# guangkun0818/speech2text

Measured on AMD Instinct MI355X. Metric: audio-seconds/sec (train step, zipformer pruned-RNN-T), higher is better.
Workload: dtype f32; 1 GPU; C3 zipformer pruned-RNN-T train step: chunk_size -1, 500 BPE, prune_range 5 (fbank+fwd+bwd+allreduce+ScaledAdam); accumulate_grad_batches=1, gemm_arith=bf16x2/3, per_gpu_batch=64, global_batch=64, labels_per_utt=50, parallelism=dp1

## Files before the change

include/s2t_mi355.h:

```cpp
#ifndef S2T_MI355_H_
#define S2T_MI355_H_

#ifdef __cplusplus
extern "C" {
#endif

int s2t_fbank_f32(const float* pcm, long pcm_stride, const long* num_samples, int batch,
                  const float* window400, const float* twiddle512, const int* mel_off,
                  const int* mel_k0, const float* mel_w, int nnz, int num_mel, float eps,
                  float scale_in, const float* cmvn_mean, const float* cmvn_istd, float* out,
                  int max_frames, long* out_frames, void* stream);

#define S2T_FBANK_CARRY_MAX 559
#define S2T_FBANK_STATE_LONGS 4
int s2t_fbank_chunk_max_frames(long chunk_samples);
int s2t_fbank_chunk_f32(const float* pcm, long pcm_stride, const long* chunk_samples, const int* flush,
                        int batch, float* carry, long* counts, const float* window400,
                        const float* twiddle512, const int* mel_off, const int* mel_k0,
                        const float* mel_w, int nnz, int num_mel, float eps, float scale_in,
                        const float* cmvn_mean, const float* cmvn_istd, float* out, int max_new_frames,
                        long* new_frames, void* stream);

#define S2T_CTC_MAX_LABELS 1023
long s2t_ctc_workspace_floats(int B, int T, int Umax);
// ... 698 lines not shown
int s2t_gemm_x3p_bal(const float* A, long lda, const unsigned short* Bp, int N, int K, float* C, long ldc,
                     int M, const float* resid, long ldr, const float* act_src, long ld_act, int act_kind,
                     int tile, float* bal_stats, float min_mean, float max_mean, float min_rms,
                     float max_rms, float grad_scale, void* stream);

typedef struct S2tRowMap {
  int hw, w;
  long sb, sh, sw, base;
} S2tRowMap;
int s2t_gemm_x3p_map(const float* A, const S2tRowMap* amap, int seg, int nseg, const long* segoff,
                     const unsigned short* Bp, int N, float* C, long ldc, const S2tRowMap* cmap,
                     long c_elems, int M, const float* bias, int tile, void* stream);

void* s2t_side_stream(void);
int s2t_stream_order(void* from, void* to);

int s2t_x3p_sample_begin(int every);
int s2t_x3p_sample_end(long* launches, double* total_ms, double* bytes, double* flops);
int s2t_x3p_sample_min_bytes(double* bytes_min);
long s2t_gemm_x3p_calls(void);
long s2t_linear_lt_calls(void);
int s2t_prof_pair_create(void** start, void** stop);
int s2t_prof_pair_arm(void* start, void* stop);
int s2t_prof_pair_consumed(void);
int s2t_prof_pair_ms(void* start, void* stop, float* ms);
int s2t_prof_pair_destroy(void* start, void* stop);


int s2t_add_f32(const float* a, const float* b, float* out, long n, void* stream);
int s2t_balancer_next_parity(void);

int s2t_bmm_lt(int mode, const float* A, const float* B, float* C, int batch, int M, int N, int K,
               void* workspace, long ws_bytes, void* stream);

#define S2T_ZL_NDEC 32
#define S2T_ZL_NWHITEN 11
typedef struct S2tZlLin {
  const float* w;
  const float* b;
  float* gw;
  float* gb;
  const unsigned short* pf;
  const unsigned short* pb;
  int N, K;
} S2tZlLin;
typedef struct S2tZlBal {
  float min_mean, max_mean, min_rms, max_rms, grad_scale;
} S2tZlBal;
typedef struct S2tZlWh {
  int groups;
  float limit, grad_scale;
} S2tZlWh;
typedef struct S2tZlFf {
  S2tZlLin in, out;
  S2tZlBal hidden;
  S2tZlWh out_wh;
  S2tZlBal post;
} S2tZlFf;
typedef struct S2tZlSa {
  S2tZlLin in, out;
  S2tZlWh wh;
} S2tZlSa;
typedef struct S2tZlConv {
  S2tZlLin in, out;
  S2tZlBal bal1, bal2;
  S2tZlWh wh;
// ... 86 lines not shown
```

speech2text_amd/csrc/gemm.hip:

```cpp
#include "common.h"
#include "../../include/s2t_mi355.h"
#include <algorithm>
#include <cstdint>
#include <cstdio>
#include <cstdlib>
#include <type_traits>

namespace {

typedef float f32x16 __attribute__((ext_vector_type(16)));
typedef float f32x2 __attribute__((ext_vector_type(2)));
typedef __bf16 bf16x2 __attribute__((ext_vector_type(2)));
typedef __bf16 bf16x8 __attribute__((ext_vector_type(8)));

__device__ __forceinline__ void split_pair(float x0, float x1, unsigned& p0, unsigned& p1,
                                           unsigned& p2) {
  f32x2 x = {x0, x1};
  p0 = __builtin_bit_cast(unsigned, __builtin_convertvector(x, bf16x2));
  f32x2 h = {__uint_as_float(p0 << 16), __uint_as_float(p0 & 0xFFFF0000u)};
  x = x - h;
  p1 = __builtin_bit_cast(unsigned, __builtin_convertvector(x, bf16x2));
  f32x2 h1 = {__uint_as_float(p1 << 16), __uint_as_float(p1 & 0xFFFF0000u)};
  x = x - h1;
  p2 = __builtin_bit_cast(unsigned, __builtin_convertvector(x, bf16x2));
// ... 39 lines not shown
  int act_kind;
  int pro_a, pro_b;
  float* colsum;
  int accumulate;
  int kper;
  int tiles_m, tiles_n;
  int splits;
  int debug;
  float alpha;
  int sym_cg;
  int tile_force;
  int wide_ep;
  Patch pt;
  const float* sq_other;
  long ld_sq;
  float* sq_sums;
  int np;
};

__device__ __forceinline__ float log1p_fast(float e) {
  const float u = 1.f + e;
  return u == 1.f ? e : __logf(u) * __fdividef(e, u - 1.f);
}
__device__ __forceinline__ float swoosh(float x, int kind) {
  const float off = kind == ACT_SWOOSH_L ? 4.f : 1.f;
  const float c = kind == ACT_SWOOSH_L ? 0.035f : 0.313261687f;
  const float z = x - off;
  return fmaxf(z, 0.f) + log1p_fast(__expf(-fabsf(z))) - 0.08f * x - c;
}
__device__ __forceinline__ float swoosh_deriv(float x, int kind) {
  const float off = kind == ACT_SWOOSH_L ? 4.f : 1.f;
  return __fdividef(1.f, 1.f + __expf(off - x)) - 0.08f;
}
template <int ROWS, bool KC, int ACT, int BK, bool PATCH = false>
struct Tile {
  static constexpr int LD = KC ? (BK + 4) : (ROWS + 4);
  static constexpr int SIZE = KC ? ROWS * LD : BK * LD;
  static constexpr int NV = ROWS * BK / 4 / 256;

  __device__ static __forceinline__ unsigned load(float4 (&v)[NV], const float* __restrict__ src,
                                                  long ld, int out0, int out_n, int k0, int k_n,
                                                  const Patch& pt) {
    unsigned ok = 0;
#pragma unroll
    for (int i = 0; i < NV; ++i) {
      const int idx = threadIdx.x + 256 * i;
      int o, k;
      if (KC) {
        o = out0 + idx / (BK / 4);
        k = k0 + 4 * (idx % (BK / 4));
      } else {
        constexpr int V = ROWS / 4;
        k = k0 + idx / V;
        o = out0 + 4 * (idx % V);
      }
      const bool valid = o < out_n && k < k_n;
      ok |= (valid ? 1u : 0u) << i;
      const int oc = min(o, KC ? out_n - 1 : out_n - 4), kc = min(k, KC ? k_n - 4 : k_n - 1);
      const float* p;
      if (PATCH)
        p = KC ? src + patch_row(pt, oc) + patch_col(pt, kc) : src + patch_row(pt, kc) + patch_col(pt, oc);
      else
        p = KC ? src + (long)oc * ld + kc : src + (long)kc * ld + oc;
      v[i] = *reinterpret_cast<const float4*>(p);
    }
    return ok;
  }
  __device__ static __forceinline__ void store(float* __restrict__ s, const float4 (&v)[NV],
                                               unsigned ok) {
#pragma unroll
    for (int i = 0; i < NV; ++i) {
      const int idx = threadIdx.x + 256 * i;
      float4 x = v[i];
      if (ACT != ACT_NONE)
        x = make_float4(swoosh(x.x, ACT), swoosh(x.y, ACT), swoosh(x.z, ACT), swoosh(x.w, ACT));
      if (!((ok >> i) & 1u)) x = make_float4(0.f, 0.f, 0.f, 0.f);
      if (KC) {
        *reinterpret_cast<float4*>(s + (idx / (BK / 4)) * LD + 4 * (idx % (BK / 4))) = x;
      } else {
        constexpr int V = ROWS / 4;
        *reinterpret_cast<float4*>(s + (idx / V) * LD + 4 * (idx % V)) = x;
      }
    }
  }
  __device__ static __forceinline__ float4 frag(const float* __restrict__ s, int t0, int sgrp,
                                                int lane) {
    const int o = t0 + (lane & 31), kb = 8 * sgrp + 4 * (lane >> 5);
    if (KC) return *reinterpret_cast<const float4*>(s + o * LD + kb);
    return make_float4(s[kb * LD + o], s[(kb + 1) * LD + o], s[(kb + 2) * LD + o],
                       s[(kb + 3) * LD + o]);
  }
};

constexpr int bk_of(int tm, int tn, int mode) {
  return BK0;
}

typedef unsigned u32x4_t __attribute__((ext_vector_type(4)));
template <int TM, int TN, int PRO, int NP = 3, bool PATCH = false>
__device__ __forceinline__ void tn_p3_body(const GemmArgs& g, const unsigned bid) {
  constexpr int BM = 64 * TM, BN = 64 * TN, BK = 32;
  __shared__ __attribute__((aligned(16))) unsigned char sA[BM * BK * 2 * NP];
  __shared__ __attribute__((aligned(16))) unsigned char sB[BN * BK * 2 * NP];
  const int total = g.tiles_m * g.tiles_n;
  const int q = (int)(bid >> 3);
  const int zslice = (int)(bid & 7) + 8 * (q / total);
  const int lin = q % total;
  if (zslice >= g.splits) return;
  const int tm = lin / g.tiles_n, tn = lin % g.tiles_n;
  const int m0 = tm * BM, n0 = tn * BN;
  if (g.sym_cg > 0) {
    if (tn < tm || n0 / g.sym_cg > (m0 + BM - 1) / g.sym_cg) return;
  }
  const int csum_tn = g.sym_cg > 0 ? tm : 0;
  const int lane = threadIdx.x & 63, wave = threadIdx.x >> 6;
  const int wm = (wave >> 1) * (BM / 2), wn = (wave & 1) * (BN / 2);
  const int kbeg = zslice * g.kper;
  const int kend = min(g.K, kbeg + g.kper);
  if (kbeg >= kend) return;
  const bool want_csum = g.colsum != nullptr && tn == csum_tn;
  const bool np3 = NP == 3 && g.np != 2;

  f32x16 acc[TM][TN];
#pragma unroll
  for (int i = 0; i < TM; ++i)
#pragma unroll
    for (int j = 0; j < TN; ++j)
#pragma unroll
      for (int r = 0; r < 16; ++r) acc[i][j][r] = 0.f;

  const int so = threadIdx.x & 63, kg = threadIdx.x >> 6;
  const unsigned sdst = (unsigned)(((((so >> 5) * 2 + (kg >> 1)) * NP) * 64 + (kg & 1) * 32 + (so & 31)) * 16);
  float ra[TM][8], rb[TN][8];
  float csum[TM];
#pragma unroll
  for (int u = 0; u < TM; ++u) csum[u] = 0.f;
#define TN3_LOAD(R, NU, SRC, LD, O0, ON, K0)                                                   \
  _Pragma("unroll") for (int u = 0; u < NU; ++u) {                                             \
    const int oc_ = min((O0) + 64 * u + so, (ON) - 1);                                         \
    _Pragma("unroll") for (int e = 0; e < 8; ++e)                                              \
      R[u][e] = (SRC)[(long)min((K0) + 8 * kg + e, kend - 1) * (LD) + oc_];                    \
  }
#define TN3_STORE(R, NU, S, O0, ON, K0, ACT, CSUM)                                             \
  _Pragma("unroll") for (int u = 0; u < NU; ++u) {                                             \
    const bool ov_ = (O0) + 64 * u + so < (ON);                                                \
    float v_[8];                                                                               \
    _Pragma("unroll") for (int e = 0; e < 8; ++e) {                                            \
      float x_ = R[u][e];                                                                      \
      if (ACT != ACT_NONE) x_ = swoosh(x_, ACT);                                               \
      v_[e] = (ov_ && (K0) + 8 * kg + e < kend) ? x_ : 0.f;                                    \
    }                                                                                          \
    if (CSUM) csum[u] += ((v_[0] + v_[1]) + (v_[2] + v_[3])) + ((v_[4] + v_[5]) + (v_[6] + v_[7])); \
    unsigned a0_, a1_, a2_, b0_, b1_, b2_, c0_, c1_, c2_, d0_, d1_, d2_;                       \
    unsigned char* d_ = (S) + u * (2 * 2 * NP * 1024) + sdst;                                   \
    if (np3) {                                                                                 \
      split_pair(v_[0], v_[1], a0_, a1_, a2_);                                                 \
      split_pair(v_[2], v_[3], b0_, b1_, b2_);                                                 \
      split_pair(v_[4], v_[5], c0_, c1_, c2_);                                                 \
      split_pair(v_[6], v_[7], d0_, d1_, d2_);                                                 \
      const u32x4_t q2_ = {a2_, b2_, c2_, d2_};                                                \
      *reinterpret_cast<u32x4_t*>(d_ + 2048) = q2_;                                            \
    } else {                                                                                   \
      split_pair2(v_[0], v_[1], a0_, a1_);                                                     \
      split_pair2(v_[2], v_[3], b0_, b1_);                                                     \
      split_pair2(v_[4], v_[5], c0_, c1_);                                                     \
      split_pair2(v_[6], v_[7], d0_, d1_);                                                     \
    }                                                                                          \
    const u32x4_t q0_ = {a0_, b0_, c0_, d0_}, q1_ = {a1_, b1_, c1_, d1_};                      \
    *reinterpret_cast<u32x4_t*>(d_) = q0_;                                                     \
    *reinterpret_cast<u32x4_t*>(d_ + 1024) = q1_;                                              \
  }
  int pcol[TN];
#pragma unroll
  for (int u = 0; u < TN; ++u) pcol[u] = PATCH ? patch_col(g.pt, min(n0 + 64 * u + so, g.N - 1)) : 0;
// ... 50 lines not shown
      acc[i][j] = __builtin_amdgcn_mfma_f32_32x32x16_bf16(pa[i][PA], pb[j][PB], acc[i][j], 0, 0, 0);
      if (np3) { S2T_P3_TERM(2, 0) S2T_P3_TERM(1, 1) S2T_P3_TERM(0, 2) }
      S2T_P3_TERM(1, 0) S2T_P3_TERM(0, 1)
      S2T_P3_TERM(0, 0)
#undef S2T_P3_TERM
    }
  }
#undef TN3_LOAD
#undef TN3_LOAD_PATCH
#undef TN3_STORE
  if (want_csum) {
    __syncthreads();
    float* red = reinterpret_cast<float*>(sA);
#pragma unroll
    for (int u = 0; u < TM; ++u) red[kg * BM + 64 * u + so] = csum[u];
    __syncthreads();
    if (threadIdx.x < BM && m0 + (int)threadIdx.x < g.M) {
      const int t = threadIdx.x;
      atomicAdd(g.colsum + m0 + t, ((red[t] + red[BM + t]) + (red[2 * BM + t] + red[3 * BM + t])) * g.alpha);
    }
  }
  if (g.debug & 1) return;
  const int hi = lane >> 5, lo = lane & 31;
#pragma unroll
  for (int i = 0; i < TM; ++i)
#pragma unroll
    for (int j = 0; j < TN; ++j) {
      const int col = n0 + wn + 32 * j + lo;
      if (col >= g.N) continue;
#pragma unroll
      for (int r = 0; r < 16; ++r) {
        const int row = m0 + wm + 32 * i + (r & 3) + 8 * (r >> 2) + 4 * hi;
        if (row >= g.M) continue;
        atomicAdd(g.C + (long)row * g.ldc + col, acc[i][j][r] * g.alpha);
      }
    }
}

__device__ __forceinline__ int tnw_perm32(int t) {
  const int a = t >> 2, mi = t & 3;
  return ((a + 2 * mi) & 7) + 8 * mi;
}
typedef float f32x4_t __attribute__((ext_vector_type(4)));
struct TnwUnit {
  const float* src;
  long ld;
  unsigned dst;
  int a, kg;
  bool valid, colok, isA;
};
template <int MI, int NJ, int PRO, bool PATCH = false>
__device__ __forceinline__ void tn_w_body(const GemmArgs& g, const unsigned bid, unsigned char* sm) {
  constexpr int BM = 64 * MI, BN = 64 * NJ, BK = 32;
  constexpr int IMG_A = BM * BK * 6, IMG_B = BN * BK * 6, BUF = IMG_A + IMG_B;
  constexpr int UNITS = BM + BN, NSLOT = (UNITS + 255) / 256;
  const int total = g.tiles_m * g.tiles_n;
  const int q = (int)(bid >> 3);
  const int zslice = (int)(bid & 7) + 8 * (q / total);
  const int lin = q % total;
  if (zslice >= g.splits) return;
  const int tm = lin / g.tiles_n, tn = lin % g.tiles_n;
  const int m0 = tm * BM, n0 = tn * BN;
  const int tid = threadIdx.x, lane = tid & 63, wave = tid >> 6;
  const bool producer = wave >= 4;
  const int kbeg = zslice * g.kper;
  const int kend = min(g.K, kbeg + g.kper);
  if (kbeg >= kend) return;
// ... 159 lines not shown
        const int kg = idx / (BM / 4), mq = idx - kg * (BM / 4);
#pragma unroll
        for (int mi = 0; mi < 4; ++mi) red[kg * BM + 4 * mq + mi] = cs[j][mi];
      }
    __syncthreads();
    if (tid < BM && m0 + tid < g.M)
      atomicAdd(g.colsum + m0 + tid, ((red[tid] + red[BM + tid]) + (red[2 * BM + tid] + red[3 * BM + tid])) * g.alpha);
  }
  if (producer || (g.debug & 1)) return;
  const int hi = lane >> 5, lo = lane & 31;
#pragma unroll
  for (int i = 0; i < MI; ++i)
#pragma unroll
    for (int j = 0; j < NJ; ++j) {
      const int c = n0 + wn + 32 * j + lo;
      if (c >= g.N) continue;
#pragma unroll
      for (int rr = 0; rr < 16; ++rr) {
        const int row = m0 + wm + 32 * i + (rr & 3) + 8 * (rr >> 2) + 4 * hi;
        if (row >= g.M) continue;
        atomicAdd(g.C + (long)row * g.ldc + c, acc[i][j][rr] * g.alpha);
      }
    }
}
template <int PRO, bool PATCH = false>
__device__ __forceinline__ void tn_w_shape(const GemmArgs& g, int shape, unsigned bid, unsigned char* sm) {
  if (shape == 1) tn_w_body<2, 3, PRO, PATCH>(g, bid, sm);
  else if (shape == 2) tn_w_body<3, 2, PRO, PATCH>(g, bid, sm);
  else tn_w_body<2, 2, PRO, PATCH>(g, bid, sm);
}
constexpr int TNW_LDS = 2 * (128 + 192) * 32 * 6;
constexpr int TNW_LDS0 = 2 * (128 + 128) * 32 * 6;

template <int TM, int TN, int MODE, int PRO, bool X3 = false, bool PATCH = false, bool P3 = false>
__device__ __forceinline__ void gemm_body(const GemmArgs& g, const unsigned bid) {
  if constexpr (P3 && X3 && MODE == MODE_TN && !PATCH) {
    tn_p3_body<TM, TN, PRO>(g, bid);
    return;
  }
  constexpr bool A_KC = MODE != MODE_TN, B_KC = MODE == MODE_NT;
  constexpr int BM = 64 * TM, BN = 64 * TN;
  constexpr int BK = bk_of(TM, TN, MODE);
  using TA = Tile<BM, A_KC, (MODE == MODE_NT ? PRO : ACT_NONE), BK, (PATCH && MODE == MODE_NT)>;
  using TB = Tile<BN, B_KC, (MODE == MODE_TN ? PRO : ACT_NONE), BK, (PATCH && MODE == MODE_TN)>;
  __shared__ __attribute__((aligned(16))) float sA[TA::SIZE];
  __shared__ __attribute__((aligned(16))) float sB[TB::SIZE];

  const int total = g.tiles_m * g.tiles_n;
  const int per_xcd = (total + 7) / 8;
  int lin, zslice = 0;
  if (MODE == MODE_TN) {
    const int q = (int)(bid >> 3);
    zslice = (int)(bid & 7) + 8 * (q / total);
    lin = q % total;
    if (zslice >= g.splits) return;
  } else {
    lin = (int)((bid & 7) * per_xcd + (bid >> 3));
    if (lin >= total) return;
  }
  const int tm = lin / g.tiles_n, tn = lin % g.tiles_n;
  const int m0 = tm * BM, n0 = tn * BN;
  if (MODE == MODE_TN && g.sym_cg > 0) {
    if (tn < tm || n0 / g.sym_cg > (m0 + BM - 1) / g.sym_cg) return;
  }
  const int csum_tn = (MODE == MODE_TN && g.sym_cg > 0) ? tm : 0;
  const int lane = threadIdx.x & 63, wave = threadIdx.x >> 6;
  const int wm = (wave >> 1) * (BM / 2), wn = (wave & 1) * (BN / 2);

  int kbeg = 0, kend = g.K;
  if (MODE == MODE_TN) {
    kbeg = zslice * g.kper;
    kend = min(g.K, kbeg + g.kper);
    if (kbeg >= kend) return;
  }

  f32x16 acc[TM][TN];
// ... 153 lines not shown
  }
#pragma unroll
  for (int i = 0; i < TM; ++i)
#pragma unroll
    for (int j = 0; j < TN; ++j) {
      const int col = n0 + wn + 32 * j + lo;
      if (col >= g.N) continue;
      const float bv = g.bias ? g.bias[col] : 0.f;
#pragma unroll
      for (int r = 0; r < 16; ++r) {
        const int row = m0 + wm + 32 * i + (r & 3) + 8 * (r >> 2) + 4 * hi;
        if (row >= g.M) continue;
        float v = acc[i][j][r];
        float* cp = g.C + (long)row * g.ldc + col;
        if (g.debug & 1) continue;
        if (MODE == MODE_TN) {
          atomicAdd(cp, v * g.alpha);
        } else {
          v += bv;
          if (g.act_src) v *= swoosh_deriv(g.act_src[(long)row * g.lds + col], g.act_kind);
          if (g.resid) v += g.resid[(long)row * g.ldr + col];
          if (g.accumulate) v += *cp;
          *cp = v;
        }
      }
    }
}

template <int TM, int TN, int MODE, int PRO, bool X3 = false, bool PATCH = false, bool P3 = false>
__global__ __launch_bounds__(256) void gemm_kernel(GemmArgs g) {
  gemm_body<TM, TN, MODE, PRO, X3, PATCH, P3>(g, blockIdx.x);
}

template <int TM, int TN, int MODE>
__global__ __launch_bounds__(256) void gemm_batched_kernel(GemmArgs g, long sA, long sB, long sC) {
  GemmArgs h = g;
  h.A += (long)blockIdx.y * sA;
  h.B += (long)blockIdx.y * sB;
  h.C += (long)blockIdx.y * sC;
  gemm_body<TM, TN, MODE, ACT_NONE, true, false, (MODE == MODE_TN)>(h, blockIdx.x);
}

constexpr int MAXG = 24;
struct TnProb {
  const float* A;
  const float* B;
  float* C;
  float* colsum;
  int lda, ldb, ldc, M, N, K, kper, tiles_m, tiles_n, splits;
  float alpha;
  int shape;
};
struct TnGroup {
  int n;
  int debug;
  int np;
  unsigned begin[MAXG + 1];
  TnProb p[MAXG];
};

template <bool X3, int TNW = 1, bool P3 = false, int TMW = 1>
__global__ __launch_bounds__(256) void gemm_tn_grouped_kernel(TnGroup grp) {
  int i = 0;
  while (i + 1 < grp.n && blockIdx.x >= grp.begin[i + 1]) ++i;
  const TnProb& q = grp.p[i];
  GemmArgs g{q.A, q.lda, q.B, q.ldb, q.C, q.ldc, q.M, q.N, q.K, nullptr, nullptr, 0, nullptr, 0,
             0, 0, 0, q.colsum, 0, q.kper, q.tiles_m, q.tiles_n, q.splits, grp.debug, q.alpha};
  g.np = grp.np;
  gemm_body<TMW, TNW, MODE_TN, ACT_NONE, X3, false, P3>(g, blockIdx.x - grp.begin[i]);
}

template <int TM, int TN, int PRO>
__global__ __launch_bounds__(256) void gemm_tn_p2_kernel(GemmArgs g) {
// ... 229 lines not shown
    return -2;
  const bool c_vec = (reinterpret_cast<uintptr_t>(C) & 15) == 0 && (sC & 3) == 0 && (ldc & 3) == 0 && (N & 3) == 0;
  if (mode == MODE_TN && !c_vec) return -2;
  if ((a_kc || b_kc) && (K & 3)) return -2;
  if ((!a_kc && (M & 3)) || (!b_kc && (N & 3))) return -2;
  if (M < 4 || N < 4 || K < 4) return -2;
  GemmArgs g{A, lda, B, ldb, C, ldc, M, N, K, nullptr, nullptr, 0, nullptr, 0, 0, 0,
             0, nullptr, 0, 0, 0, 0, 0, 0, 1.f, 0};
  hipStream_t st = (hipStream_t)stream;
  g.np = s2t_gemm_arith();
  g.tiles_m = (M + 63) / 64;
  g.tiles_n = (N + 63) / 64;
  const int total = g.tiles_m * g.tiles_n;
  if (mode == MODE_TN) {
    int splits = std::max(1, std::min(8, K / (2 * KR)));
    int kper = (K + splits - 1) / splits;
    kper = ((kper + KR - 1) / KR) * KR;
    g.kper = kper;
    g.splits = (K + kper - 1) / kper;
    const unsigned grid = (unsigned)(8 * total * ((g.splits + 7) / 8));
    hipLaunchKernelGGL((gemm_batched_kernel<1, 1, MODE_TN>), dim3(grid, batch), dim3(256), 0, st, g, sA, sB, sC);
  } else {
    g.splits = 1;
    g.wide_ep = c_vec;
    const unsigned grid = (unsigned)(((total + 7) / 8) * 8);
    if (mode == MODE_NT)
      hipLaunchKernelGGL((gemm_batched_kernel<1, 1, MODE_NT>), dim3(grid, batch), dim3(256), 0, st, g, sA, sB, sC);
    else
      hipLaunchKernelGGL((gemm_batched_kernel<1, 1, MODE_NN>), dim3(grid, batch), dim3(256), 0, st, g, sA, sB, sC);
  }
  return (int)hipGetLastError();
}

extern "C" int s2t_gemm_f32_tiled(int mode, const float* A, long lda, const float* B, long ldb,
                                  float* C, long ldc, int M, int N, int K, const float* bias,
                                  const float* resid, long ldr, int tile, void* stream) {
  if (M <= 0 || N <= 0 || K <= 0 || (mode != MODE_NT && mode != MODE_NN)) return -1;
  if (tile != 0 && tile != 11 && tile != 12 && tile != 21 && tile != 22 && tile != 23) return -1;
  const bool b_kc = mode == MODE_NT;
  if ((reinterpret_cast<uintptr_t>(A) & 15) || (reinterpret_cast<uintptr_t>(B) & 15) || (lda & 3) ||
      (ldb & 3) || (K & 3) || (!b_kc && (N & 3)) || M < 4 || N < 4 || K < 4)
    return -2;
  GemmArgs g{A, lda, B, ldb, C, ldc, M, N, K, bias, resid, ldr, nullptr, 0, 0, 0,
             0, nullptr, 0, 0, 0, 0, 0, 0, 1.f, 0, tile};
  hipStream_t st = (hipStream_t)stream;
  return mode == MODE_NT ? dispatch<MODE_NT>(g, st) : dispatch<MODE_NN>(g, st);
}

extern "C" int s2t_conv3x3_gemm(int mode, const float* x, int B, int H, int W, int C, int sh, int sw,
                                int CO, const float* w2_or_g, const float* bias, float* out,
                                float* db, void* stream) {
  if (B <= 0 || H < 3 || W < 3 || C <= 0 || CO <= 0 || sh <= 0 || sw <= 0 || (mode != 0 && mode != 2))
    return -1;
  const int Ho = (H - 3) / sh + 1, Wo = (W - 3) / sw + 1;
  const long R = (long)B * Ho * Wo, nx = (long)B * H * W * C;
  if ((C & 3) || (CO & 3) || nx >= (1L << 31) || R >= (1L << 31) || R < 4) return -2;
  if ((reinterpret_cast<uintptr_t>(x) & 15) || (reinterpret_cast<uintptr_t>(w2_or_g) & 15) ||
      (reinterpret_cast<uintptr_t>(out) & 15))
    return -2;
  const Patch pt{3 * C, Ho * Wo, Wo, H * W * C, sh * W * C, sw * C, W * C};
  const int K9 = 9 * C;
  hipStream_t st = (hipStream_t)stream;
  if (mode == 0) {
    GemmArgs g{x, 0, w2_or_g, K9, out, CO, (int)R, CO, K9, bias, nullptr, 0, nullptr, 0, 0, 0,
               0, nullptr, 0, 0, 0, 0, 0, 0, 1.f, 0, 0, 0, pt};
    g.np = s2t_gemm_arith_of(0);
// ... 183 lines not shown
```

speech2text_amd/csrc/gemm_lib.hip:

```cpp
#include <hip/hip_runtime.h>
#include <hipblaslt/hipblaslt.h>

#include <cmath>
#include <cstdio>
#include <cstdlib>
#include <cstring>
#include <map>
#include <mutex>
#include <tuple>

extern "C" int s2t_gemm_f32(int mode, const float* A, long lda, const float* B, long ldb, float* C,
                            long ldc, int M, int N, int K, const float* bias, const float* resid,
                            long ldr, const float* act_src, long lds, int act_kind, int pro_a,
                            int pro_b, float* colsum, int accumulate, void* stream);
extern "C" int s2t_nn_x3(int set);
extern "C" int s2t_gemm_f32_tiled(int mode, const float* A, long lda, const float* B, long ldb,
                                  float* C, long ldc, int M, int N, int K, const float* bias,
                                  const float* resid, long ldr, int tile, void* stream);

namespace {

constexpr int MAX_CAND = 16;

constexpr float OWN_MARGIN = 0.97f;
// ... 17 lines not shown
  int ncand = 0;
  bool tuned = false;
  bool own = false;
  int own_tile = 0;
};

using Key = std::tuple<int, int, int, int, long, long, long, long, int>;
std::map<Key, Plan> g_plans;
using BKey = std::tuple<int, int, int, int, int>;
struct Winner {
  hipblasLtMatmulAlgo_t algo;
  bool own;
  int own_tile;
};
std::map<BKey, Winner> g_winner;
int g_tunings = 0;
long g_own_calls = 0;
constexpr size_t MAX_PLANS = 8192;

constexpr int TUNE_BUDGET = 192;

int half_octave(int m) { return (int)std::floor(2.0 * std::log2((double)(m < 1 ? 1 : m))); }

void destroy_plan(Plan& p) {
  if (p.a) hipblasLtMatrixLayoutDestroy(p.a);
  if (p.b) hipblasLtMatrixLayoutDestroy(p.b);
  if (p.c) hipblasLtMatrixLayoutDestroy(p.c);
  if (p.d) hipblasLtMatrixLayoutDestroy(p.d);
  if (p.desc) hipblasLtMatmulDescDestroy(p.desc);
}
std::mutex g_mu;
hipblasLtHandle_t g_handle = nullptr;
long g_lt_calls = 0;

#define LT_CHECK(x)                                   \
  do {                                                \
    hipblasStatus_t s__ = (x);                        \
    if (s__ != HIPBLAS_STATUS_SUCCESS) return -100 - (int)s__; \
  } while (0)

int make_plan(Plan& p, int mode, int M, int N, int K, long ldx, long ldw, long ldc, long ldd,
              bool has_bias, size_t ws_bytes) {
  if (!g_handle) LT_CHECK(hipblasLtCreate(&g_handle));
  LT_CHECK(hipblasLtMatmulDescCreate(&p.desc, HIPBLAS_COMPUTE_32F, HIP_R_32F));
  hipblasOperation_t opa = mode == 0 ? HIPBLAS_OP_T : HIPBLAS_OP_N, opb = HIPBLAS_OP_N;
  LT_CHECK(hipblasLtMatmulDescSetAttribute(p.desc, HIPBLASLT_MATMUL_DESC_TRANSA, &opa, sizeof(opa)));
  LT_CHECK(hipblasLtMatmulDescSetAttribute(p.desc, HIPBLASLT_MATMUL_DESC_TRANSB, &opb, sizeof(opb)));
  if (has_bias) {
    hipblasLtEpilogue_t epi = HIPBLASLT_EPILOGUE_BIAS;
    LT_CHECK(hipblasLtMatmulDescSetAttribute(p.desc, HIPBLASLT_MATMUL_DESC_EPILOGUE, &epi, sizeof(epi)));
  }
  const int out_rows = mode == 0 ? N : K;
  const int inner = mode == 0 ? K : N;
  LT_CHECK(hipblasLtMatrixLayoutCreate(&p.a, HIP_R_32F, K, N, ldw));
  LT_CHECK(hipblasLtMatrixLayoutCreate(&p.b, HIP_R_32F, inner, M, ldx));
  LT_CHECK(hipblasLtMatrixLayoutCreate(&p.c, HIP_R_32F, out_rows, M, ldc));
  LT_CHECK(hipblasLtMatrixLayoutCreate(&p.d, HIP_R_32F, out_rows, M, ldd));
  hipblasLtMatmulPreference_t pref;
  LT_CHECK(hipblasLtMatmulPreferenceCreate(&pref));
  LT_CHECK(hipblasLtMatmulPreferenceSetAttribute(pref, HIPBLASLT_MATMUL_PREF_MAX_WORKSPACE_BYTES,
                                                 &ws_bytes, sizeof(ws_bytes)));
  int n = 0;
  hipblasStatus_t st = hipblasLtMatmulAlgoGetHeuristic(g_handle, p.desc, p.a, p.b, p.c, p.d, pref,
                                                       MAX_CAND, p.cand, &n);
  hipblasLtMatmulPreferenceDestroy(pref);
  if (st != HIPBLAS_STATUS_SUCCESS || n < 1) return -2;
// ... 142 lines not shown
    if (w != g_winner.end()) {
      p.tuned = true;
      p.own = w->second.own;
      p.own_tile = w->second.own_tile;
      for (int i = 0; i < p.ncand; ++i)
        if (p.cand[i].workspaceSize <= (size_t)ws_bytes &&
            memcmp(&p.cand[i].algo, &w->second.algo, sizeof(hipblasLtMatmulAlgo_t)) == 0) {
          p.algo = p.cand[i].algo;
          p.ws = p.cand[i].workspaceSize;
          break;
        }
    } else if (g_tunings < TUNE_BUDGET) {
      tune(p, X, W, C == D ? nullptr : C, C == D ? 0.f : beta, (long)M * ldd, workspace,
           (size_t)ws_bytes, (hipStream_t)stream, mode, ldx, ldw, bias, ldc, ldd, M, N, K);
      g_winner.emplace(bkey, Winner{p.algo, p.own, p.own_tile});
      ++g_tunings;
    } else {
      p.tuned = true;
    }
  }
  if (p.own && (beta == 0.f || (beta == 1.f && C != D)) &&
      run_own(mode, X, ldx, W, ldw, bias, C, ldc, beta, D, ldd, M, N, K, p.own_tile,
              (hipStream_t)stream) == 0) {
    ++g_own_calls;
    return 0;
  }
  const float alpha = 1.f;
  LT_CHECK(hipblasLtMatmul(g_handle, p.desc, &alpha, W, p.a, X, p.b, &beta, C, p.c, D, p.d, &p.algo,
                           workspace, p.ws, (hipStream_t)stream));
  return 0;
}

extern "C" long s2t_linear_lt_calls(void) { return g_lt_calls; }
extern "C" long s2t_linear_lt_own_calls(void) { return g_own_calls; }

namespace {
struct BPlan {
  hipblasLtMatmulDesc_t desc = nullptr;
  hipblasLtMatrixLayout_t a = nullptr, b = nullptr, d = nullptr;
  hipblasLtMatmulAlgo_t algo;
  size_t ws = 0;
  bool ok = false;
};
using BmmKey = std::tuple<int, int, int, int, int>;
std::map<BmmKey, BPlan> g_bplans;

int set_batch(hipblasLtMatrixLayout_t l, int batch, long stride) {
  int32_t bc = batch;
  int64_t so = stride;
  LT_CHECK(hipblasLtMatrixLayoutSetAttribute(l, HIPBLASLT_MATRIX_LAYOUT_BATCH_COUNT, &bc, sizeof(bc)));
  LT_CHECK(hipblasLtMatrixLayoutSetAttribute(l, HIPBLASLT_MATRIX_LAYOUT_STRIDED_BATCH_OFFSET, &so, sizeof(so)));
  return 0;
}

int make_bplan(BPlan& p, int mode, int M, int N, int K, int batch, size_t ws_bytes) {
  if (!g_handle) LT_CHECK(hipblasLtCreate(&g_handle));
  LT_CHECK(hipblasLtMatmulDescCreate(&p.desc, HIPBLAS_COMPUTE_32F, HIP_R_32F));
  hipblasOperation_t opa = mode == 0 ? HIPBLAS_OP_T : HIPBLAS_OP_N;
  hipblasOperation_t opb = mode == 2 ? HIPBLAS_OP_T : HIPBLAS_OP_N;
  LT_CHECK(hipblasLtMatmulDescSetAttribute(p.desc, HIPBLASLT_MATMUL_DESC_TRANSA, &opa, sizeof(opa)));
  LT_CHECK(hipblasLtMatmulDescSetAttribute(p.desc, HIPBLASLT_MATMUL_DESC_TRANSB, &opb, sizeof(opb)));
  if (mode == 0) LT_CHECK(hipblasLtMatrixLayoutCreate(&p.a, HIP_R_32F, K, N, K));
  else LT_CHECK(hipblasLtMatrixLayoutCreate(&p.a, HIP_R_32F, N, K, N));
  if (mode == 2) LT_CHECK(hipblasLtMatrixLayoutCreate(&p.b, HIP_R_32F, M, K, M));
  else LT_CHECK(hipblasLtMatrixLayoutCreate(&p.b, HIP_R_32F, K, M, K));
  LT_CHECK(hipblasLtMatrixLayoutCreate(&p.d, HIP_R_32F, N, M, N));
// ... 4 lines not shown
  rc = set_batch(p.d, batch, (long)M * N);
  if (rc) return rc;
  hipblasLtMatmulPreference_t pref;
  LT_CHECK(hipblasLtMatmulPreferenceCreate(&pref));
  LT_CHECK(hipblasLtMatmulPreferenceSetAttribute(pref, HIPBLASLT_MATMUL_PREF_MAX_WORKSPACE_BYTES,
                                                 &ws_bytes, sizeof(ws_bytes)));
  hipblasLtMatmulHeuristicResult_t res[4];
  int n = 0;
  hipblasStatus_t st = hipblasLtMatmulAlgoGetHeuristic(g_handle, p.desc, p.a, p.b, p.d, p.d, pref, 4, res, &n);
  hipblasLtMatmulPreferenceDestroy(pref);
  if (st != HIPBLAS_STATUS_SUCCESS || n < 1) return -2;
  p.algo = res[0].algo;
  p.ws = res[0].workspaceSize;
  p.ok = true;
  return 0;
}
}

extern "C" int s2t_bmm_lt(int mode, const float* A, const float* B, float* C, int batch, int M, int N,
                          int K, void* workspace, long ws_bytes, void* stream) {
  if (batch <= 0 || M <= 0 || N <= 0 || K <= 0 || mode < 0 || mode > 2 || !A || !B || !C) return -1;
  std::lock_guard<std::mutex> lock(g_mu);
  const BmmKey key{mode, M, N, K, batch};
  auto it = g_bplans.find(key);
  if (it == g_bplans.end()) {
    if (g_bplans.size() >= 512) return -2;
    BPlan p;
    const int rc = make_bplan(p, mode, M, N, K, batch, (size_t)ws_bytes);
    it = g_bplans.emplace(key, p).first;
    if (rc != 0 && rc != -2) return rc;
  }
  BPlan& p = it->second;
  if (!p.ok || p.ws > (size_t)ws_bytes) return -2;
  const float alpha = 1.f, beta = 0.f;
  LT_CHECK(hipblasLtMatmul(g_handle, p.desc, &alpha, B, p.a, A, p.b, &beta, C, p.d, C, p.d, &p.algo,
                           workspace, p.ws, (hipStream_t)stream));
  return 0;
}
```

speech2text_amd/csrc/zip_layer.hip:

```cpp
#include <hip/hip_runtime.h>

#include <cmath>
#include <cstdint>
#include <cstdio>
#include <cstring>
#include <atomic>
#include <functional>
#include <mutex>
#include <unordered_map>
#include <vector>

#include "../../include/s2t_mi355.h"
#include "common.h"

namespace {

constexpr int kMagic = 0x5a4c3532;
constexpr float kPenLimit = 25.0f;
constexpr int kMaxProb = 48;

thread_local char g_err[256] = "";

std::mutex g_mu;
float* g_pin = nullptr;
// ... 230 lines not shown
  if (e.bal) {
    float* t = c.ar.alloc(n);
    Epi plain;
    TRY(lt_matmul(c, mode, x, ldx, R, L, plain, t));
    return balancer_bwd(c, *e.bal, e.act_src, cols, t, cols, R, cols, out, cols, kSwOff[e.act_kind], e.bal_stats);
  }
  float* y = out;
  float* tmp = nullptr;
  if (e.act_src) y = tmp = c.ar.alloc(n);
  if (!c.dry) {
    const float* res = e.act_src ? nullptr : e.resid2;
    int rc = s2t_linear_lt(mode, x, ldx, L.w, L.K, e.bias, res, cols, res ? 1.0f : 0.0f, y, cols, (int)R, L.N,
                           L.K, c.c.lt_ws, c.c.lt_ws_bytes, (void*)c.st);
    if (rc == -2)
      rc = s2t_gemm_f32(mode, x, ldx, L.w, L.K, y, cols, (int)R, cols, inner, e.bias, res, cols, nullptr, 0, 0, 0,
                        0, nullptr, 0, (void*)c.st);
    if (rc != 0) return fail(rc, "s2t_linear_lt");
  }
  if (e.act_src) {
    RUN(s2t_swoosh_bwd(e.act_src, tmp, out, n, kSwOff[e.act_kind], (void*)c.st));
    if (e.resid2) RUN(s2t_add_f32(out, e.resid2, out, n, (void*)c.st));
  }
  if (e.act2 == 3) {
    RUN(s2t_add_f32(out, e.resid_b, e.out2, n, (void*)c.st));
  } else {
    if (e.resid_b) RUN(s2t_add_f32(out, e.resid_b, out, n, (void*)c.st));
    if (e.act2) RUN(s2t_swoosh_fwd(out, e.out2, n, kSwOff[e.act2], kSwC[e.act2], (void*)c.st));
  }
  return 0;
}

int bmm(Ctx& c, int mode, const float* a, const float* b, float* out, int n, int M, int N, int K) {
  if (c.dry) return 0;
  const int mn = M < N ? (M < K ? M : K) : (N < K ? N : K);
  if (mode != 2 && K % 4 == 0 && (mode == 0 || N % 4 == 0) && mn >= 4) {
    const long lda = K, sA = (long)M * K;
    const long ldb = mode == 0 ? K : N, sB = (long)N * K;
    const int rc = s2t_gemm_f32_batched(mode, a, lda, sA, b, ldb, sB, out, N, (long)M * N, M, N, K, n, (void*)c.st);
    if (rc == 0) return 0;
    if (rc != -2) return fail(rc, "s2t_gemm_f32_batched");
  }
  RUN(s2t_bmm_lt(mode, a, b, out, n, M, N, K, c.c.lt_ws, c.c.lt_ws_bytes, (void*)c.st));
  return 0;
}

const S2tZlWhScratch* wh_scratch(const Ctx& c, int C) {
  for (int i = 0; i < c.c.nwh; ++i)
    if (c.c.wh[i].C == C) return &c.c.wh[i];
  return nullptr;
}

int whiten_stats(Ctx& c, WStat& s, const float* x, long ldx, long R, int C, int groups) {
  s.on = 1;
  s.G = groups;
  s.cg = C / groups;
  s.cov = c.ar.alloc((long)groups * s.cg * s.cg);
  s.mean = c.ar.alloc(C);
  s.scal = c.ar.alloc(4);
  const S2tZlWhScratch* sc0 = wh_scratch(c, C);
  const bool fused = c.c.whiten_x3p == 2 && C >= 16 && (C & 7) == 0 && s.cg <= 1024 &&
                     R >= 4 && R * C * 4 < 0x7FFFFF00L && R * ldx * 4 < 0x7FFFFF00L && sc0 && sc0->tab;
  s.pieces = nullptr;
  if (fused) {
    s.dcov = c.ar.alloc((long)C * C);
    s.bias = c.ar.alloc(C);
    s.sums = c.ar.alloc(128);
    s.pieces = reinterpret_cast<unsigned short*>(c.ar.alloc((s2t_x3p_plane_elems(C, C) + 1) / 2));
  }
  s.pg = (fused && c.c.whiten_fwd_pg) ? c.ar.alloc(R * C) : nullptr;
  if (c.dry) return 0;
  const S2tZlWhScratch* sc = wh_scratch(c, C);
  if (!sc) return fail(-1, "whiten_stats: no scratch for this channel count");
  if ((ldx & 3) || (C & 3) || R < 4 || (reinterpret_cast<uintptr_t>(x) & 15))
    return fail(-1, "whiten_stats: layout outside the TN kernel's rules");
  s.host = pinned_slot();
// ... 723 lines not shown
```

speech2text_amd/zip_kernels.py:

```python
import ctypes
import os

import torch
import torch.nn.functional as F

from . import _native as N
from . import flat
from . import planes

_SW = {True: (4.0, 0.035), False: (1.0, 0.313261687)}


def _dev(*ts):
    for t in ts:
        if t is not None and not t.is_cuda:
            raise RuntimeError("speech2text_amd zipformer kernels run on the GPU only "
                               "(no CPU fallback); got a CPU tensor")


def _c16(t):
    t = t.contiguous()
    if t.data_ptr() % 16:
        t = t.clone()
    return t
# ... 1078 lines not shown
    if not (wparam.is_leaf and flat.owned(wparam) and _tn_ok(g2) and _tn_ok(a2)):
        return False
    wg = wparam.grad
    if wg is None or not wg.is_contiguous() or wg.dim() < 2:
        return False
    if wg.dim() > 2:
        wg = wg.view(wg.shape[0], -1)
    bg = None
    if bparam is not None:
        if not (bparam.is_leaf and flat.owned(bparam)):
            return False
        bg = bparam.grad
        if bg is None or not bg.is_contiguous():
            return False
    st = None
    if 2.0 * g2.shape[0] * g2.shape[1] * a2.shape[1] >= 2.0e10:
        st = _side_launch_stream(g2, a2)
    gemm_tn(g2, a2, wg, bg, pro, stream=st)
    if notify:
        flat.grad_written(wparam)
        if bparam is not None:
            flat.grad_written(bparam)
    return True


def batched_matmul(mode, a, b, own_tn=False):
    n = a.shape[0]
    if mode == 0:
        M, K, Nn = a.shape[1], a.shape[2], b.shape[1]
    elif mode == 1:
        M, K, Nn = a.shape[1], a.shape[2], b.shape[2]
    else:
        M, K, Nn = a.shape[2], a.shape[1], b.shape[2]
    tn_ok = own_tn and mode == 2 and M % 4 == 0 and Nn % 4 == 0
    if ((mode != 2 or tn_ok) and (mode == 2 or K % 4 == 0) and (mode == 0 or Nn % 4 == 0)
            and min(M, Nn, K) >= 4 and a.is_cuda and a.dtype is torch.float32 and b.dtype is torch.float32
            and a.is_contiguous() and b.is_contiguous() and n > 0):
        out = (torch.zeros if mode == 2 else torch.empty)((n, M, Nn), dtype=torch.float32, device=a.device)
        N.PROF[0] and N.profile_note("s2t_gemm_f32_batched", 4.0 * (a.numel() + b.numel() + out.numel()),
                                     2.0 * n * M * Nn * K)
        rc = N.lib().s2t_gemm_f32_batched(mode, N.fp(a), a.stride(1), a.stride(0), N.fp(b), b.stride(1),
                                          b.stride(0), N.fp(out), Nn, M * Nn, M, Nn, K, n, N.stream())
        if rc == 0:
            return out
        if rc != -2:
            N.check(rc, "s2t_gemm_f32_batched")
    if a.is_cuda and a.dtype is torch.float32 and b.dtype is torch.float32 and a.is_contiguous() \
            and b.is_contiguous() and n > 0:
        out = torch.empty((n, M, Nn), dtype=torch.float32, device=a.device)
        ws = _lt_workspace(a.device)
        N.PROF[0] and N.profile_note("s2t_bmm_lt", 4.0 * (a.numel() + b.numel() + out.numel()), 2.0 * n * M * Nn * K)
        rc = N.lib().s2t_bmm_lt(mode, N.fp(a), N.fp(b), N.fp(out), n, M, Nn, K, ws.data_ptr(), ws.numel(),
                                N.stream())
        if rc == 0:
            return out
        if rc != -2:
            N.check(rc, "s2t_bmm_lt")
    if mode == 0:
        return torch.bmm(a, b.transpose(1, 2))
    if mode == 1:
        return torch.bmm(a, b)
    return torch.bmm(a.transpose(1, 2), b)


TnProblem = N.struct("S2tTnProblem")


def wgrad_group(items):
    ok = []
    for it in items:
        w, b, g2, a2 = it[:4]
        alpha = it[4] if len(it) > 4 else 1.0
        wg = w.grad
        if (_tn_ok(g2) and _tn_ok(a2) and flat.owned(w) and wg is not None and wg.is_contiguous()
                and (b is None or (flat.owned(b) and b.grad is not None))):
            ok.append((w, b, g2, a2, alpha))
            continue
        if alpha != 1.0 or not wgrad_into(w, b, g2, a2, 0, notify=True):
            dw, db = linear_wgrad(g2, a2, b is not None)
            w.grad.add_(dw.view(w.shape), alpha=alpha)
            flat.grad_written(w)
            if b is not None:
                b.grad.add_(db, alpha=alpha)
                flat.grad_written(b)
    n = len(ok)
    if n == 0:
        return
    arr = (TnProblem * n)()
    nbytes = flops = 0.0
    for q, (w, b, g2, a2, alpha) in zip(arr, ok):
# ... 834 lines not shown
```

Baseline: 18190 audio-seconds/sec.

## Route batched matmuls through own split-bf16 kernels instead of hipBLASLt

```diff
diff --git a/include/s2t_mi355.h b/include/s2t_mi355.h
--- a/include/s2t_mi355.h
+++ b/include/s2t_mi355.h
@@ -754,6 +754,10 @@
 
 int s2t_bmm_lt(int mode, const float* A, const float* B, float* C, int batch, int M, int N, int K,
                void* workspace, long ws_bytes, void* stream);
+long s2t_bmm_lt_calls(void);
+
+int s2t_bmm_f32(int mode, const float* A, const float* B, float* C, int batch, int M, int N, int K,
+                void* workspace, long ws_bytes, void* stream);
 
 #define S2T_ZL_NDEC 32
 #define S2T_ZL_NWHITEN 11
diff --git a/speech2text_amd/csrc/gemm.hip b/speech2text_amd/csrc/gemm.hip
--- a/speech2text_amd/csrc/gemm.hip
+++ b/speech2text_amd/csrc/gemm.hip
@@ -95,7 +95,7 @@
   const float off = kind == ACT_SWOOSH_L ? 4.f : 1.f;
   return __fdividef(1.f, 1.f + __expf(off - x)) - 0.08f;
 }
-template <int ROWS, bool KC, int ACT, int BK, bool PATCH = false>
+template <int ROWS, bool KC, int ACT, int BK, bool PATCH = false, bool UNAL = false>
 struct Tile {
   static constexpr int LD = KC ? (BK + 4) : (ROWS + 4);
   static constexpr int SIZE = KC ? ROWS * LD : BK * LD;
@@ -105,6 +105,22 @@
                                                   long ld, int out0, int out_n, int k0, int k_n,
                                                   const Patch& pt) {
     unsigned ok = 0;
+    if constexpr (UNAL) {
+      static_assert(KC && !PATCH && NV <= 8, "the dword-aligned loader serves k-contiguous operands");
+      typedef unsigned int u32x4 __attribute__((ext_vector_type(4)));
+      const __amdgpu_buffer_rsrc_t rs =
+          __builtin_amdgcn_make_buffer_rsrc(const_cast<float*>(src), 0, out_n * (int)ld * 4, 0x00020000);
+#pragma unroll
+      for (int i = 0; i < NV; ++i) {
+        const int idx = threadIdx.x + 256 * i;
+        const int o = out0 + idx / (BK / 4), k = k0 + 4 * (idx % (BK / 4));
+#pragma unroll
+        for (int e = 0; e < 4; ++e) ok |= ((o < out_n && k + e < k_n) ? 1u : 0u) << (4 * i + e);
+        const u32x4 q = __builtin_amdgcn_raw_buffer_load_b128(rs, (o < out_n && k < k_n) ? (o * (int)ld + k) * 4 : 0, 0, 0);
+        v[i] = make_float4(__uint_as_float(q.x), __uint_as_float(q.y), __uint_as_float(q.z), __uint_as_float(q.w));
+      }
+      return ok;
+    }
 #pragma unroll
     for (int i = 0; i < NV; ++i) {
       const int idx = threadIdx.x + 256 * i;
@@ -137,7 +153,12 @@
       float4 x = v[i];
       if (ACT != ACT_NONE)
         x = make_float4(swoosh(x.x, ACT), swoosh(x.y, ACT), swoosh(x.z, ACT), swoosh(x.w, ACT));
-      if (!((ok >> i) & 1u)) x = make_float4(0.f, 0.f, 0.f, 0.f);
+      if constexpr (UNAL) {
+        const unsigned m = ok >> (4 * i);
+        x = make_float4((m & 1u) ? x.x : 0.f, (m & 2u) ? x.y : 0.f, (m & 4u) ? x.z : 0.f, (m & 8u) ? x.w : 0.f);
+      } else if (!((ok >> i) & 1u)) {
+        x = make_float4(0.f, 0.f, 0.f, 0.f);
+      }
       if (KC) {
         *reinterpret_cast<float4*>(s + (idx / (BK / 4)) * LD + 4 * (idx % (BK / 4))) = x;
       } else {
@@ -160,7 +181,7 @@
 }
 
 typedef unsigned u32x4_t __attribute__((ext_vector_type(4)));
-template <int TM, int TN, int PRO, int NP = 3, bool PATCH = false>
+template <int TM, int TN, int PRO, int NP = 3, bool PATCH = false, bool STORE = false>
 __device__ __forceinline__ void tn_p3_body(const GemmArgs& g, const unsigned bid) {
   constexpr int BM = 64 * TM, BN = 64 * TN, BK = 32;
   __shared__ __attribute__((aligned(16))) unsigned char sA[BM * BK * 2 * NP];
@@ -201,8 +222,13 @@
 #define TN3_LOAD(R, NU, SRC, LD, O0, ON, K0)                                                   \
   _Pragma("unroll") for (int u = 0; u < NU; ++u) {                                             \
     const int oc_ = min((O0) + 64 * u + so, (ON) - 1);                                         \
-    _Pragma("unroll") for (int e = 0; e < 8; ++e)                                              \
-      R[u][e] = (SRC)[(long)min((K0) + 8 * kg + e, kend - 1) * (LD) + oc_];                    \
+    if (STORE && (K0) + BK <= kend) {                                                          \
+      const float* p_ = (SRC) + (long)((K0) + 8 * kg) * (LD) + oc_;                            \
+      _Pragma("unroll") for (int e = 0; e < 8; ++e) R[u][e] = p_[(long)e * (LD)];              \
+    } else {                                                                                   \
+      _Pragma("unroll") for (int e = 0; e < 8; ++e)                                            \
+        R[u][e] = (SRC)[(long)min((K0) + 8 * kg + e, kend - 1) * (LD) + oc_];                  \
+    }                                                                                          \
   }
 #define TN3_STORE(R, NU, S, O0, ON, K0, ACT, CSUM)                                             \
   _Pragma("unroll") for (int u = 0; u < NU; ++u) {                                             \
@@ -319,7 +345,8 @@
       for (int r = 0; r < 16; ++r) {
         const int row = m0 + wm + 32 * i + (r & 3) + 8 * (r >> 2) + 4 * hi;
         if (row >= g.M) continue;
-        atomicAdd(g.C + (long)row * g.ldc + col, acc[i][j][r] * g.alpha);
+        if constexpr (STORE) g.C[(long)row * g.ldc + col] = acc[i][j][r] * g.alpha;
+        else atomicAdd(g.C + (long)row * g.ldc + col, acc[i][j][r] * g.alpha);
       }
     }
 }
@@ -545,7 +572,7 @@
 constexpr int TNW_LDS = 2 * (128 + 192) * 32 * 6;
 constexpr int TNW_LDS0 = 2 * (128 + 128) * 32 * 6;
 
-template <int TM, int TN, int MODE, int PRO, bool X3 = false, bool PATCH = false, bool P3 = false>
+template <int TM, int TN, int MODE, int PRO, bool X3 = false, bool PATCH = false, bool P3 = false, bool AU = false>
 __device__ __forceinline__ void gemm_body(const GemmArgs& g, const unsigned bid) {
   if constexpr (P3 && X3 && MODE == MODE_TN && !PATCH) {
     tn_p3_body<TM, TN, PRO>(g, bid);
@@ -554,7 +581,7 @@
   constexpr bool A_KC = MODE != MODE_TN, B_KC = MODE == MODE_NT;
   constexpr int BM = 64 * TM, BN = 64 * TN;
   constexpr int BK = bk_of(TM, TN, MODE);
-  using TA = Tile<BM, A_KC, (MODE == MODE_NT ? PRO : ACT_NONE), BK, (PATCH && MODE == MODE_NT)>;
+  using TA = Tile<BM, A_KC, (MODE == MODE_NT ? PRO : ACT_NONE), BK, (PATCH && MODE == MODE_NT), AU>;
   using TB = Tile<BN, B_KC, (MODE == MODE_TN ? PRO : ACT_NONE), BK, (PATCH && MODE == MODE_TN)>;
   __shared__ __attribute__((aligned(16))) float sA[TA::SIZE];
   __shared__ __attribute__((aligned(16))) float sB[TB::SIZE];
@@ -774,13 +801,21 @@
   gemm_body<TM, TN, MODE, PRO, X3, PATCH, P3>(g, blockIdx.x);
 }
 
-template <int TM, int TN, int MODE>
+template <int TM, int TN, int MODE, bool AU = false>
 __global__ __launch_bounds__(256) void gemm_batched_kernel(GemmArgs g, long sA, long sB, long sC) {
   GemmArgs h = g;
   h.A += (long)blockIdx.y * sA;
   h.B += (long)blockIdx.y * sB;
   h.C += (long)blockIdx.y * sC;
-  gemm_body<TM, TN, MODE, ACT_NONE, true, false, (MODE == MODE_TN)>(h, blockIdx.x);
+  gemm_body<TM, TN, MODE, ACT_NONE, true, false, (MODE == MODE_TN), AU>(h, blockIdx.x);
+}
+template <int TM, int TN>
+__global__ __launch_bounds__(256) void bmm_tn_store_kernel(GemmArgs g, long sA, long sB, long sC) {
+  GemmArgs h = g;
+  h.A += (long)blockIdx.y * sA;
+  h.B += (long)blockIdx.y * sB;
+  h.C += (long)blockIdx.y * sC;
+  tn_p3_body<TM, TN, ACT_NONE, 3, false, true>(h, blockIdx.x * 8u);
 }
 
 constexpr int MAXG = 24;
@@ -1076,6 +1111,78 @@
   return (int)hipGetLastError();
 }
 
+constexpr int BMM_K1 = 512, BMM_K2 = 2048;
+namespace {
+constexpr long BMM_WIDE_WG = 256;
+bool bmm_wide(int batch, int M) { return (long)batch * ((M + 63) / 64) >= BMM_WIDE_WG; }
+int bmm_tile_n(int batch, int M, int N) {
+  const int tn = N <= 64 ? 1 : (N <= 128 ? 2 : 3);
+  return bmm_wide(batch, M) ? tn : 1;
+}
+bool bmm_depth_ok(int batch, int M, int K) { return K <= BMM_K1 || (K <= BMM_K2 && bmm_wide(batch, M)); }
+template <int TM, int TN>
+int bmm_nn_au(GemmArgs g, int batch, long sA, long sB, long sC, hipStream_t st) {
+  g.tiles_m = (g.M + 64 * TM - 1) / (64 * TM);
+  g.tiles_n = (g.N + 64 * TN - 1) / (64 * TN);
+  const unsigned grid = (unsigned)(((g.tiles_m * g.tiles_n + 7) / 8) * 8);
+  hipLaunchKernelGGL((gemm_batched_kernel<TM, TN, MODE_NN, true>), dim3(grid, batch), dim3(256), 0, st, g, sA, sB, sC);
+  return (int)hipGetLastError();
+}
+template <int TM, int TN>
+int bmm_tn_store(GemmArgs g, int batch, long sA, long sB, long sC, hipStream_t st) {
+  g.tiles_m = (g.M + 64 * TM - 1) / (64 * TM);
+  g.tiles_n = (g.N + 64 * TN - 1) / (64 * TN);
+  hipLaunchKernelGGL((bmm_tn_store_kernel<TM, TN>), dim3((unsigned)(g.tiles_m * g.tiles_n), batch), dim3(256), 0, st,
+                     g, sA, sB, sC);
+  return (int)hipGetLastError();
+}
+}
+extern "C" int s2t_bmm_f32(int mode, const float* A, const float* B, float* C, int batch, int M, int N,
+                           int K, void* workspace, long ws_bytes, void* stream) {
+  if (batch <= 0 || M <= 0 || N <= 0 || K <= 0 || mode < 0 || mode > 2 || !A || !B || !C) return -1;
+  const auto al16 = [](const void* p) { return (reinterpret_cast<uintptr_t>(p) & 15) == 0; };
+  const auto al4 = [](const void* p) { return (reinterpret_cast<uintptr_t>(p) & 3) == 0; };
+  const long sA = (long)M * K, sB = (long)N * K, sC = (long)M * N;
+  hipStream_t st = (hipStream_t)stream;
+  if (batch <= 65535 && al4(A) && al4(B) && al4(C)) {
+    if (mode != MODE_TN && M >= 4 && N >= 4 && K >= 4) {
+      const long lda = K, ldb = mode == MODE_NT ? K : N;
+      const bool b_ok = al16(B) && !(ldb & 3) && !(sB & 3);
+      if (b_ok && al16(A) && !(K & 3) && !(sA & 3)) {
+        const int rc = s2t_gemm_f32_batched(mode, A, lda, sA, B, ldb, sB, C, N, sC, M, N, K, batch, stream);
+        if (rc != -2) return rc;
+      } else if (b_ok && mode == MODE_NN && bmm_depth_ok(batch, M, K) &&
+                 ((long)M + 64) * K * 4 < (1L << 31)) {
+        GemmArgs g{A, lda, B, ldb, C, N, M, N, K, nullptr, nullptr, 0, nullptr, 0, 0, 0,
+                   0, nullptr, 0, 0, 0, 0, 0, 0, 1.f, 0};
+        g.np = s2t_gemm_arith();
+        g.splits = 1;
+        g.wide_ep = al16(C) && !(sC & 3) && !(N & 3);
+        switch (bmm_tile_n(batch, M, N)) {
+          case 2: return bmm_nn_au<1, 2>(g, batch, sA, sB, sC, st);
+          case 3: return bmm_nn_au<1, 3>(g, batch, sA, sB, sC, st);
+          default: return bmm_nn_au<1, 1>(g, batch, sA, sB, sC, st);
+        }
+      }
+    }
+    if (mode == MODE_TN) {
+      if (bmm_depth_ok(batch, M, K)) {
+        GemmArgs g{A, M, B, N, C, N, M, N, K, nullptr, nullptr, 0, nullptr, 0, 0, 0,
+                   0, nullptr, 0, 0, 0, 0, 0, 0, 1.f, 0};
+        g.np = s2t_gemm_arith();
+        g.splits = 1;
+        g.kper = ((K + KR - 1) / KR) * KR;
+        switch (bmm_tile_n(batch, M, N)) {
+          case 2: return bmm_tn_store<1, 2>(g, batch, sA, sB, sC, st);
+          case 3: return bmm_tn_store<1, 3>(g, batch, sA, sB, sC, st);
+          default: return bmm_tn_store<1, 1>(g, batch, sA, sB, sC, st);
+        }
+      }
+    }
+  }
+  return s2t_bmm_lt(mode, A, B, C, batch, M, N, K, workspace, ws_bytes, stream);
+}
+
 extern "C" int s2t_gemm_f32_tiled(int mode, const float* A, long lda, const float* B, long ldb,
                                   float* C, long ldc, int M, int N, int K, const float* bias,
                                   const float* resid, long ldr, int tile, void* stream) {
diff --git a/speech2text_amd/csrc/gemm_lib.hip b/speech2text_amd/csrc/gemm_lib.hip
--- a/speech2text_amd/csrc/gemm_lib.hip
+++ b/speech2text_amd/csrc/gemm_lib.hip
@@ -73,6 +73,7 @@
 std::mutex g_mu;
 hipblasLtHandle_t g_handle = nullptr;
 long g_lt_calls = 0;
+long g_bmm_lt_calls = 0;
 
 #define LT_CHECK(x)                                   \
   do {                                                \
@@ -281,6 +282,7 @@
 }
 
 extern "C" long s2t_linear_lt_calls(void) { return g_lt_calls; }
+extern "C" long s2t_bmm_lt_calls(void) { return g_bmm_lt_calls; }
 extern "C" long s2t_linear_lt_own_calls(void) { return g_own_calls; }
 
 namespace {
@@ -351,6 +353,7 @@
   }
   BPlan& p = it->second;
   if (!p.ok || p.ws > (size_t)ws_bytes) return -2;
+  ++g_bmm_lt_calls;
   const float alpha = 1.f, beta = 0.f;
   LT_CHECK(hipblasLtMatmul(g_handle, p.desc, &alpha, B, p.a, A, p.b, &beta, C, p.d, C, p.d, &p.algo,
                            workspace, p.ws, (hipStream_t)stream));
diff --git a/speech2text_amd/csrc/zip_layer.hip b/speech2text_amd/csrc/zip_layer.hip
--- a/speech2text_amd/csrc/zip_layer.hip
+++ b/speech2text_amd/csrc/zip_layer.hip
@@ -286,15 +286,7 @@
 
 int bmm(Ctx& c, int mode, const float* a, const float* b, float* out, int n, int M, int N, int K) {
   if (c.dry) return 0;
-  const int mn = M < N ? (M < K ? M : K) : (N < K ? N : K);
-  if (mode != 2 && K % 4 == 0 && (mode == 0 || N % 4 == 0) && mn >= 4) {
-    const long lda = K, sA = (long)M * K;
-    const long ldb = mode == 0 ? K : N, sB = (long)N * K;
-    const int rc = s2t_gemm_f32_batched(mode, a, lda, sA, b, ldb, sB, out, N, (long)M * N, M, N, K, n, (void*)c.st);
-    if (rc == 0) return 0;
-    if (rc != -2) return fail(rc, "s2t_gemm_f32_batched");
-  }
-  RUN(s2t_bmm_lt(mode, a, b, out, n, M, N, K, c.c.lt_ws, c.c.lt_ws_bytes, (void*)c.st));
+  RUN(s2t_bmm_f32(mode, a, b, out, n, M, N, K, c.c.lt_ws, c.c.lt_ws_bytes, (void*)c.st));
   return 0;
 }
 
diff --git a/speech2text_amd/zip_kernels.py b/speech2text_amd/zip_kernels.py
--- a/speech2text_amd/zip_kernels.py
+++ b/speech2text_amd/zip_kernels.py
@@ -1134,11 +1134,10 @@
         M, K, Nn = a.shape[1], a.shape[2], b.shape[2]
     else:
         M, K, Nn = a.shape[2], a.shape[1], b.shape[2]
-    tn_ok = own_tn and mode == 2 and M % 4 == 0 and Nn % 4 == 0
-    if ((mode != 2 or tn_ok) and (mode == 2 or K % 4 == 0) and (mode == 0 or Nn % 4 == 0)
-            and min(M, Nn, K) >= 4 and a.is_cuda and a.dtype is torch.float32 and b.dtype is torch.float32
-            and a.is_contiguous() and b.is_contiguous() and n > 0):
-        out = (torch.zeros if mode == 2 else torch.empty)((n, M, Nn), dtype=torch.float32, device=a.device)
+    dense = a.is_cuda and a.dtype is torch.float32 and b.dtype is torch.float32 and a.is_contiguous() \
+        and b.is_contiguous() and n > 0
+    if own_tn and mode == 2 and M % 4 == 0 and Nn % 4 == 0 and min(M, Nn, K) >= 4 and dense:
+        out = torch.zeros((n, M, Nn), dtype=torch.float32, device=a.device)
         N.PROF[0] and N.profile_note("s2t_gemm_f32_batched", 4.0 * (a.numel() + b.numel() + out.numel()),
                                      2.0 * n * M * Nn * K)
         rc = N.lib().s2t_gemm_f32_batched(mode, N.fp(a), a.stride(1), a.stride(0), N.fp(b), b.stride(1),
@@ -1147,17 +1146,16 @@
             return out
         if rc != -2:
             N.check(rc, "s2t_gemm_f32_batched")
-    if a.is_cuda and a.dtype is torch.float32 and b.dtype is torch.float32 and a.is_contiguous() \
-            and b.is_contiguous() and n > 0:
+    if dense:
         out = torch.empty((n, M, Nn), dtype=torch.float32, device=a.device)
         ws = _lt_workspace(a.device)
-        N.PROF[0] and N.profile_note("s2t_bmm_lt", 4.0 * (a.numel() + b.numel() + out.numel()), 2.0 * n * M * Nn * K)
-        rc = N.lib().s2t_bmm_lt(mode, N.fp(a), N.fp(b), N.fp(out), n, M, Nn, K, ws.data_ptr(), ws.numel(),
-                                N.stream())
+        N.PROF[0] and N.profile_note("s2t_bmm_f32", 4.0 * (a.numel() + b.numel() + out.numel()), 2.0 * n * M * Nn * K)
+        rc = N.lib().s2t_bmm_f32(mode, N.fp(a), N.fp(b), N.fp(out), n, M, Nn, K, ws.data_ptr(), ws.numel(),
+                                 N.stream())
         if rc == 0:
             return out
         if rc != -2:
-            N.check(rc, "s2t_bmm_lt")
+            N.check(rc, "s2t_bmm_f32")
     if mode == 0:
         return torch.bmm(a, b.transpose(1, 2))
     if mode == 1:
```

After: 18180 audio-seconds/sec. No clear change (-0.1%).
